# alessiodevoto/peekvit

Measured on AMD Instinct MI355X. Metric: images/sec ViT-B/16 fwd @ batch 2048, 224x224, higher is better.
Workload: dtype f16; 1 GPU; vit_b_16 forward, batch 2048/GPU, 224x224; global_batch=2048, parallelism=replicas x1 (batch-sharded, no collective), precision_mode=auto, streams=1, operands=IEEE fp16 operands, fp32 accumulate (same MFMA rate as bf16), range-guarded, range_guard_fallbacks=0

## Files before the change

### peekvit_amd/_build.py

```python
from __future__ import annotations

import glob
import os
import subprocess
import sys

HERE = os.path.dirname(os.path.abspath(__file__))
CSRC = os.path.join(HERE, "csrc")
LIB = os.path.join(HERE, "libpeekvit_hip.so")
LIB_F16 = os.path.join(HERE, "libpeekvit_hip_f16.so")
HIPCC = os.environ.get("HIPCC", "/opt/rocm/bin/hipcc")
FLAGS = ["--offload-arch=gfx950", "-O3", "-std=c++17", "-fPIC", "-Wno-unused-result"]
HEADERS = ("peekvit_hip.h", "peekvit_hip_moe.h", "peekvit_hip_ee.h", "peekvit_hip_sparse.h", "peekvit_hip_pct.h",
           "peekvit_hip_pct_train.h", "peekvit_hip_attn_stream.h", "peekvit_hip_pct_block.h", "peekvit_hip_rank_train.h", "peekvit_hip_rank_infer.h",
           "peekvit_hip_avit_train.h", "peekvit_hip_sparse_train.h", "peekvit_hip_avit_pack_train.h", "peekvit_hip_dropout.h", "peekvit_hip_sparse_long.h",
           "peekvit_hip_sparse_long_train.h", "peekvit_hip_avit_long.h")
FILE_FLAGS = {"pv_attention.hip": ["-mllvm", "-amdgpu-mfma-vgpr-form=1"], "pv_rowops.hip": ["-fno-slp-vectorize"],
              "pv_attention_stream.hip": ["-mllvm", "-amdgpu-mfma-vgpr-form=1"],
              "pv_ee.hip": ["-fno-slp-vectorize"],
              "pv_sparse.hip": ["-fno-slp-vectorize"],
              "pv_sparse_long.hip": ["-fno-slp-vectorize"],
              "pv_pct.hip": ["-fno-slp-vectorize"],
              "pv_pct_train.hip": ["-fno-slp-vectorize"],
              "pv_rank_train.hip": ["-fno-slp-vectorize"],
              "pv_avit_train.hip": ["-fno-slp-vectorize"],
              "pv_avit_pack_train.hip": ["-fno-slp-vectorize"],
              "pv_avit_long.hip": ["-fno-slp-vectorize"],
              "pv_dropout.hip": ["-fno-slp-vectorize"],
              "pv_sparse_train.hip": ["-fno-slp-vectorize", "-mllvm", "-amdgpu-mfma-vgpr-form=1"],
              "pv_sparse_long_train.hip": ["-fno-slp-vectorize"]}


def sources():
    return sorted(glob.glob(os.path.join(CSRC, "*.hip")))


def _stale() -> bool:
    if not os.path.exists(LIB) or not os.path.exists(LIB_F16):
        return True
    t = min(os.path.getmtime(LIB), os.path.getmtime(LIB_F16))
    deps = sources() + glob.glob(os.path.join(CSRC, "*.h")) + [os.path.join(os.path.dirname(HERE), "include", h) for h in HEADERS] + [os.path.abspath(__file__)]
    return any(os.path.getmtime(d) > t for d in deps)


def build(force: bool = False, verbose: bool = False) -> str:
    if not force and not _stale():
        return LIB
    procs = []
    variants = [("build", [], LIB), ("build_f16", ["-DPV_OPERAND_F16"], LIB_F16)]
    objs = {lib: [] for _, _, lib in variants}
    for sub, defs, lib in variants:
        objdir = os.path.join(HERE, sub)
        os.makedirs(objdir, exist_ok=True)
        for src in sources():
            obj = os.path.join(objdir, os.path.basename(src)[:-4] + ".o")
            objs[lib].append(obj)
            cmd = [HIPCC, *FLAGS, *FILE_FLAGS.get(os.path.basename(src), []), *defs, "-c", src, "-o", obj]
            if verbose:
                print(" ".join(cmd))
            procs.append((src, subprocess.Popen(cmd, stdout=subprocess.PIPE, stderr=subprocess.STDOUT)))
    for src, p in procs:
        out, _ = p.communicate()
        if p.returncode != 0:
            raise RuntimeError(f"hipcc failed on {src}:\n{out.decode(errors='replace')}")
    for _, _, lib in variants:
        cmd = [HIPCC, "--offload-arch=gfx950", "-shared", "-fPIC", "-o", lib, *objs[lib]]
        r = subprocess.run(cmd, stdout=subprocess.PIPE, stderr=subprocess.STDOUT)
        if r.returncode != 0:
            raise RuntimeError(f"link failed:\n{r.stdout.decode(errors='replace')}")
    return LIB


def build_variant(tag: str, defs, force: bool = False) -> str:
    lib = os.path.join(HERE, f"libpeekvit_hip_{tag}.so")
    deps = sources() + glob.glob(os.path.join(CSRC, "*.h")) + [os.path.join(os.path.dirname(HERE), "include", h) for h in HEADERS]
    if not force and os.path.exists(lib) and all(os.path.getmtime(d) <= os.path.getmtime(lib) for d in deps):
        return lib
    objdir = os.path.join(HERE, "build_" + tag)
    os.makedirs(objdir, exist_ok=True)
    procs, objs = [], []
    for src in sources():
        obj = os.path.join(objdir, os.path.basename(src)[:-4] + ".o")
        objs.append(obj)
        procs.append((src, subprocess.Popen([HIPCC, *FLAGS, *FILE_FLAGS.get(os.path.basename(src), []), *defs, "-c", src, "-o", obj],
                                            stdout=subprocess.PIPE, stderr=subprocess.STDOUT)))
    for src, p in procs:
        out, _ = p.communicate()
        if p.returncode != 0:
            raise RuntimeError(f"hipcc failed on {src}:\n{out.decode(errors='replace')}")
    r = subprocess.run([HIPCC, "--offload-arch=gfx950", "-shared", "-fPIC", "-o", lib, *objs], stdout=subprocess.PIPE, stderr=subprocess.STDOUT)
    if r.returncode != 0:
        raise RuntimeError(f"link failed:\n{r.stdout.decode(errors='replace')}")
    return lib


if __name__ == "__main__":
    print(build(force="--force" in sys.argv, verbose=True))
```

### peekvit_amd/_lib.py

```python
from __future__ import annotations

import ctypes as C
import os
import threading

import torch

from ._build import LIB

_i64, _f32, _p, _i32 = C.c_int64, C.c_float, C.c_void_p, C.c_int32

PV_EPI_BIAS_BF16, PV_EPI_BIAS_GELU_BF16, PV_EPI_BIAS_RES_F32, PV_EPI_BIAS_POS_F32 = 0, 1, 2, 3
PV_EPI_BIAS_F32, PV_EPI_BIAS_GELU_SPLIT_BF16 = 4, 5
PV_EPI_BIAS_GELU_PAIR_BF16, PV_EPI_GELU_GRAD_BF16 = 6, 7
PV_WS_TRANSPOSE_COLSUM, PV_WS_COLSUM, PV_WS_LAYERNORM_BWD, PV_WS_GEMM_COLSUM_PARTIAL, PV_WS_GEMM_SPLITK = 1, 2, 3, 4, 5


class GemmArgs(C.Structure):
    _fields_ = [("struct_size", C.c_uint64), ("A", _p), ("W", _p), ("bias", _p), ("out", _p), ("res", _p), ("row_scale", _p), ("pos", _p),
                ("M", _i64), ("N", _i64), ("K", _i64), ("lda", _i64), ("ldw", _i64), ("ldo", _i64), ("ldr", _i64),
                ("rows_per_img_in", _i64), ("rows_per_img_out", _i64), ("row_off", _i64), ("qcols", _i64),
                ("qscale", _f32), ("epilogue", _i32),
                ("ln_gamma", _p), ("ln_beta", _p), ("ln_row_scale", _p), ("ln_out", _p), ("ln_eps", _f32),
                ("ksplit", _i32), ("colsum_partial", _p),
# ... 86 lines not shown
    "pv_layernorm_f32_bf16": (C.c_int, [_p, _i64, _p, _p, _p, _p, _i64, _i64, _i64, _f32, _p]),
    "pv_mean_pool_f32": (C.c_int, [_p, _p, _i64, _i64, _i64, _p]),
    "pv_pct_head_f32": (C.c_int, [_p, _p, _p, _p, _p, _p, _p, _p, _i64, _i64, _i64, _i64, _p]),
}

SIGNATURES_PCT_TRAIN = {
    "pv_arpe_knn": (C.c_int, [_p, _p, _i64, _i64, _i64, _p]),
    "pv_arpe_pair_moments": (C.c_int, [_p, _p, _p, _p, _i64, _i64, _i64, _p]),
    "pv_arpe_pair_max": (C.c_int, [_p, _p, _p, _p, _p, _p, _p, _p, _i64, _i64, _i64, _p]),
    "pv_arpe_pair_bwd": (C.c_int, [_p, _p, _p, _p, _p, _p, _p, _i64, _i64, _p]),
}

SIGNATURES_ATTN_STREAM = {
    "pv_attention_stream_lse_bf16": (C.c_int, [_p, _p, _p, _i64, _i64, _i64, _i64, _p, _p]),
    "pv_attention_stream_bwd_bf16": (C.c_int, [_p, _p, _p, _p, _p, _p, _i64, _i64, _i64, _i64, _f32, _p]),
}

SIGNATURES_PCT_BLOCK = {
    "pv_layernorm_bwd_sum": (C.c_int, [_p, _p, _p, _p, _p, _p, _p, _p, _i64, _i64, _i64, _f32, C.c_int, _p]),
    "pv_attention_stream_bwd16_bf16": (C.c_int, [_p, _p, _p, _p, _p, _p, _p, _i64, _i64, _i64, _i64, _f32, _p]),
}

SIGNATURES_RANK_TRAIN = {
    "pv_rank_pack_f32": (C.c_int, [_p, _p, _p, _i64, _i64, _i64, _i64, _p]),
    "pv_rank_expand_f32": (C.c_int, [_p, _p, _i64, _i64, _i64, _i64, _p]),
    "pv_rank_reduce_f32": (C.c_int, [_p, _p, _i64, _i64, _i64, _i64, _p]),
    "pv_rank_unpack_grad_f32": (C.c_int, [_p, _p, _p, _i64, _i64, _i64, _i64, _p]),
    "pv_layernorm_f32_bf16_masked": (C.c_int, [_p, _p, _p, _p, _p, _p, _i64, _i64, _f32, _p]),
    "pv_layernorm_bwd_sum_masked": (C.c_int, [_p, _p, _p, _p, _p, _p, _p, _p, _p, _i64, _i64, _i64, _f32, C.c_int, _p]),
    "pv_attention_stream_lse_w_bf16": (C.c_int, [_p, _p, _p, _i64, _i64, _i64, _i64, _f32, _p, _p]),
    "pv_attention_stream_bwd16_w_bf16": (C.c_int, [_p, _p, _p, _p, _p, _p, _p, _i64, _i64, _i64, _i64, _f32, _f32, _p]),
}

SIGNATURES_RANK_INFER = {
    "pv_rank_order_gap": (C.c_int, [_p, _p, _p, _i64, _i64, _i64, _p]),
    "pv_layernorm_gather_f32_bf16": (C.c_int, [_p, _p, _p, _p, _p, _p, _i64, _i64, _i64, _i64, _f32, _p]),
}

SIGNATURES_AVIT_TRAIN = {
    "pv_avit_act_fwd": (C.c_int, [_p] * 16 + [_i64, _i64, _i64, _i64, _f32, _f32, _f32, C.c_int, _p]),
    "pv_avit_act_bwd": (C.c_int, [_p] * 9 + [_i64, _i64, _i64, _i64, _f32, C.c_int, _p]),
}

SIGNATURES_SPARSE_TRAIN = {
    "pv_attention_varlen_w_lse_bf16": (C.c_int, [_p, _p, _p, _p, _p, _i64, _i64, _i64, _i64, _p, _p]),
    "pv_attention_varlen_w_bwd16_bf16": (C.c_int, [_p, _p, _p, _p, _p, _p, _p, _p, _p, _i64, _i64, _i64, _i64, _f32, _p]),
    "pv_residual_pack_step_train": (C.c_int, [_p, _p, _p, _p, _i64, _i64, _i64, _p, _p, _p, _p, _f32, _f32, _p,
                                              _p, _p, _p, _p, _p, _p, _p, _p, _p, _p, _p, _f32, _p, _p, _p, _p]),
    "pv_residual_pack_step_bwd": (C.c_int, [_p] * 11 + [_i64, _i64, _i64, _p, _p, _f32, _p, _p, _p, _p, _p, _p]),
}

SIGNATURES_AVIT_PACK_TRAIN = {
    "pv_avit_pack_step_train": (C.c_int, [_p] * 4 + [_i64] * 4 + [_p] * 12 + [_i64, _p, _f32, _f32, _f32, C.c_int] + [_p] * 11),
    "pv_avit_pack_step_bwd": (C.c_int, [_p] * 16 + [_i64] * 6 + [_f32, C.c_int, _p]),
}

_u64 = C.c_uint64
SIGNATURES_DROPOUT = {
    "pv_dropout_keep_u8": (C.c_int, [_p, _u64, _u64, _i64, _i64, _f32, _p]),
    "pv_dropout_f32": (C.c_int, [_p, _p, _u64, _u64, _i64, _i64, _f32, _p]),
    "pv_dropout_residual": (C.c_int, [_p, _p, _p, _u64, _u64, _i64, _i64, _f32, _p]),
    "pv_dropout_bwd16": (C.c_int, [_p, _p, _u64, _u64, _i64, _i64, _f32, _p]),
    "pv_attention_stream_lse_drop_bf16": (C.c_int, [_p, _p, _p, _i64, _i64, _i64, _i64, _f32, _u64, _u64, _p, _p]),
    "pv_attention_stream_bwd16_drop_bf16": (C.c_int, [_p, _p, _p, _p, _p, _p, _p, _i64, _i64, _i64, _i64, _f32, _f32, _u64, _u64, _p]),
}

SIGNATURES_SPARSE_LONG = {
    "pv_attention_varlen_w_stream_bf16": SIGNATURES_SPARSE["pv_attention_varlen_w_bf16"],
    "pv_residual_pack_step_long": SIGNATURES_SPARSE["pv_residual_pack_step"],
}

SIGNATURES_SPARSE_LONG_TRAIN = {
    "pv_attention_varlen_w_stream_lse_bf16": SIGNATURES_SPARSE_TRAIN["pv_attention_varlen_w_lse_bf16"],
    "pv_attention_varlen_w_stream_bwd16_bf16": SIGNATURES_SPARSE_TRAIN["pv_attention_varlen_w_bwd16_bf16"],
    "pv_residual_pack_step_long_train": SIGNATURES_SPARSE_TRAIN["pv_residual_pack_step_train"],
    "pv_residual_pack_step_long_bwd": SIGNATURES_SPARSE_TRAIN["pv_residual_pack_step_bwd"],
}

SIGNATURES_AVIT_LONG = {
    "pv_avit_pack_step_long": SIGNATURES_AVIT_PACK_TRAIN["pv_avit_pack_step_train"],
    "pv_avit_pack_step_long_bwd": SIGNATURES_AVIT_PACK_TRAIN["pv_avit_pack_step_bwd"],
}

ABI_VERSION = 10
_lock = threading.Lock()
_libs: dict = {}

_OPERAND_DEFAULT = "bf16"
_tls = threading.local()
LIB_F16 = os.path.join(os.path.dirname(os.path.abspath(__file__)), "libpeekvit_hip_f16.so")


def current_operand() -> str:
    return getattr(_tls, "operand", _OPERAND_DEFAULT)


def set_operand(op: str) -> str:
    old = current_operand()
    _tls.operand = op
    return old


def __getattr__(name):
    if name == "OPERAND":
        return current_operand()
    raise AttributeError(f"module {__name__!r} has no attribute {name!r}")


def operand_dtype():
    import torch as _t
    return _t.float16 if current_operand() == "f16" else _t.bfloat16


class PeekvitHipError(RuntimeError):
    pass


def lib_path(operand: str = "bf16") -> str:
    return LIB_F16 if operand == "f16" else LIB


def load(operand=None):
    op = current_operand() if operand is None else operand
    lib = _libs.get(op)
    if lib is not None:
        return lib
    with _lock:
        lib = _libs.get(op)
        if lib is not None:
            return lib
        path = lib_path(op)
        if not os.path.exists(path):
            raise PeekvitHipError(
                f"{path} not found: the MI355X kernels are not built. Run `python -m peekvit_amd._build` "
                "(or __graft_entry__.build()); there is no fallback path.")
        lib = C.CDLL(path)
        for name, (res, args) in {**SIGNATURES, **SIGNATURES_MOE, **SIGNATURES_EE, **SIGNATURES_SPARSE, **SIGNATURES_PCT,
                                   **SIGNATURES_PCT_TRAIN, **SIGNATURES_ATTN_STREAM, **SIGNATURES_PCT_BLOCK, **SIGNATURES_RANK_TRAIN,
                                   **SIGNATURES_RANK_INFER, **SIGNATURES_AVIT_TRAIN, **SIGNATURES_SPARSE_TRAIN, **SIGNATURES_AVIT_PACK_TRAIN,
                                   **SIGNATURES_DROPOUT, **SIGNATURES_SPARSE_LONG, **SIGNATURES_SPARSE_LONG_TRAIN,
                                   **SIGNATURES_AVIT_LONG}.items():
            fn = getattr(lib, name)
            fn.restype, fn.argtypes = res, args
        if lib.pv_version() != ABI_VERSION:
            raise PeekvitHipError(f"{path} has ABI v{lib.pv_version()}, this package binds v{ABI_VERSION}: rebuild (python -m peekvit_amd._build)")
        if lib.pv_gemm_args_size() != C.sizeof(GemmArgs):
            raise PeekvitHipError(f"{path}: pv_gemm_args is {lib.pv_gemm_args_size()} bytes in the library, {C.sizeof(GemmArgs)} in this binding")
        if lib.pv_operand_type() != (1 if op == "f16" else 0):
            raise PeekvitHipError(f"{path} was built for a different operand type")
        _libs[op] = lib
    return lib


def check(code: int, what: str = "") -> None:
    if code != 0:
        msg = load().pv_error_string(code).decode()
        raise PeekvitHipError(f"{what}: {msg} (code {code})" if what else f"{msg} (code {code})")
```

### peekvit_amd/engine.py

```python
from __future__ import annotations

import math
import os
import threading
import warnings
import weakref
from typing import Dict, List, Optional, Tuple

import torch
from torch import nn

from . import _lib, autograph, ops
import contextlib

from ._lib import (PV_EPI_BIAS_BF16, PV_EPI_BIAS_F32, PV_EPI_BIAS_GELU_BF16, PV_EPI_BIAS_GELU_SPLIT_BF16, PV_EPI_BIAS_POS_F32,
                   PV_EPI_BIAS_RES_F32, PeekvitHipError)

_MODE_DEFAULT = os.environ.get("PEEKVIT_AMD_PRECISION", "auto")
_MODES = ("auto", "bf16", "f16", "bf16x3")
if _MODE_DEFAULT not in _MODES:
    raise ValueError(f"PEEKVIT_AMD_PRECISION={_MODE_DEFAULT!r}: expected one of {_MODES}")
_lib._OPERAND_DEFAULT = "f16" if _MODE_DEFAULT == "f16" else "bf16"
_mode_tls = threading.local()

# ... 867 lines not shown
        part = workspace.get("fold_part", (nt, R, 2), torch.float32, dev)
        mlp_hyb = layer_mlp_is_hybrid()
        ops.gemm(att, bf16_weight(mha.out_proj.weight), _f32(mha.out_proj.bias), x1.view(R, D), PV_EPI_BIAS_RES_F32, M=R, res=x.view(R, D),
                 x16_out=None if mlp_hyb else x16, rowstat_out=None if mlp_hyb else part)
        if mlp_hyb:
            _mlp_half_split(blk, x1, out, R, eps, None)
            return out
        wg, c1, c2 = _fold_weights(blk.mlp.fc1.weight, blk.mlp.fc1.bias, blk.ln_2)
        stat = ops.rowstat_finalize(part, D, blk.ln_2.eps, workspace.get("fold_stat", (R, 2), torch.float32, dev))
        ops.gemm(x16, wg, None, g, PV_EPI_BIAS_GELU_BF16, M=R, fold=(stat, c1, c2))
        emit = next_ln is not None and next_ln.normalized_shape == (D,)
        o16 = workspace.get("fold_o16", (R, D), _lib.operand_dtype(), dev) if emit else None
        opart = workspace.get("fold_opart", (nt, R, 2), torch.float32, dev) if emit else None
        rowsq = workspace.get("rowsq", (nt, R), torch.float32, dev) if (next_ranks and not emit and _FUSE_RANK_NORM) else None
        ops.gemm(g, bf16_weight(blk.mlp.fc2.weight), _f32(blk.mlp.fc2.bias), out.view(R, D), PV_EPI_BIAS_RES_F32, M=R, res=x1.view(R, D),
                 x16_out=o16, rowstat_out=opart, rowsq_out=rowsq)
        if emit:
            out._pv_fold = (o16, opart, _ln_key(next_ln), _tver(out))
        if rowsq is not None:
            out._pv_rowsq = (rowsq, _tver(out))
        return out

    if hyb:
        if res_scaled:
            raise PeekvitHipError("block_forward(res_scaled=True) cannot run a hybrid layer: pass the masked tokens")
        _attention_half_split(blk, x, att, B, S, eps, row_scale)
    else:
        if h1 is not None and h1.shape == (R, D):
            h = h1
        elif handoff is not None and row_scale is None and handoff[1] == _ln_key(blk.ln_1) and handoff[0].shape == (R, D):
            h = handoff[0]
        else:
            h = workspace.get("h", (R, D), _lib.operand_dtype(), dev)
            ops.layernorm_bf16(x, _f32(blk.ln_1.weight), _f32(blk.ln_1.bias), eps, h, row_scale)
        ops.gemm(h, bf16_weight(mha.in_proj_weight), _f32(mha.in_proj_bias), qkv, PV_EPI_BIAS_BF16, M=R,
                 qcols=D, qscale=float(dh) ** -0.5)
        ops.attention(qkv, att, B, S, H, dh)
    mlp_hyb = layer_mlp_is_hybrid()
    if mlp_hyb and res_scaled:
        raise PeekvitHipError("block_forward(res_scaled=True) cannot run a layer whose MLP half is in split precision: pass the masked tokens")
    fuse2 = _ln_fusable(D, D) and not mlp_hyb
    if res_scaled and (h1 is None or row_scale is None or fuse2):
        raise PeekvitHipError("block_forward(res_scaled=True) needs row_scale, the caller's h1 and the tile GEMM (no full-row LayerNorm fusion)")
    if fuse2 or row_scale is not None:
        ops.gemm(att, bf16_weight(mha.out_proj.weight), _f32(mha.out_proj.bias), x1.view(R, D), PV_EPI_BIAS_RES_F32, M=R,
                 res=x.view(R, D), row_scale=row_scale, res_scaled=res_scaled,
                 ln=(_f32(blk.ln_2.weight), _f32(blk.ln_2.bias), eps, h2, row_scale) if fuse2 else None)
        ln2_done = fuse2
    else:
        ln2_done = _residual_gemm(att, bf16_weight(mha.out_proj.weight), _f32(mha.out_proj.bias), x1.view(R, D), x.view(R, D), R,
                                  ln=(_f32(blk.ln_2.weight), _f32(blk.ln_2.bias), eps, h2))
    if mlp_hyb:
        _mlp_half_split(blk, x1, out, R, eps, row_scale)
        return out
    if not ln2_done:
        ops.layernorm_bf16(x1, _f32(blk.ln_2.weight), _f32(blk.ln_2.bias), eps, h2, row_scale)
    _act_gemm(h2, bf16_weight(blk.mlp.fc1.weight), _f32(blk.mlp.fc1.bias), g, R, gelu=True)
    fuse_next = next_ln is not None and _ln_fusable(D, M) and next_ln.normalized_shape == (D,)
    hn = workspace.get("h", (R, D), _lib.operand_dtype(), dev) if fuse_next else None
    rowsq = None
    if next_ranks and not fuse_next and _FUSE_RANK_NORM and ops.gemm_tile_rows(R, D, M, PV_EPI_BIAS_RES_F32) == 256:
        rowsq = workspace.get("rowsq", ((D + 255) // 256, R), torch.float32, dev)
    if fuse_next or rowsq is not None:
        ops.gemm(g, bf16_weight(blk.mlp.fc2.weight), _f32(blk.mlp.fc2.bias), out.view(R, D), PV_EPI_BIAS_RES_F32, M=R,
                 res=x1.view(R, D), rowsq_out=rowsq,
                 ln=(_f32(next_ln.weight), _f32(next_ln.bias), next_ln.eps, hn, None) if fuse_next else None)
    else:
        want = next_ln is not None and next_ln.normalized_shape == (D,)
        hn = workspace.get("h", (R, D), _lib.operand_dtype(), dev) if want else None
        fuse_next = _residual_gemm(g, bf16_weight(blk.mlp.fc2.weight), _f32(blk.mlp.fc2.bias), out.view(R, D), x1.view(R, D), R,
                                   ln=(_f32(next_ln.weight), _f32(next_ln.bias), next_ln.eps, hn) if want else None)
    if fuse_next:
        out._pv_ln = (hn, _ln_key(next_ln))
    if rowsq is not None:
        out._pv_rowsq = (rowsq, _tver(out))
    return out


_LAST_BLOCK_ROWS = os.environ.get("PEEKVIT_AMD_LAST_BLOCK_ROWS", "1") != "0"
_GATE_LN1 = os.environ.get("PEEKVIT_AMD_GATE_LN1", "1") != "0"
_GATE_NO_MASKED = os.environ.get("PEEKVIT_AMD_GATE_MASKED", "0") != "1"


def rows_only_ok(blk: nn.Module) -> bool:
    import torch.nn.modules.module as _m
    if not _LAST_BLOCK_ROWS or _mode() == "bf16x3" or layer_is_hybrid() or layer_mlp_is_hybrid():
        return False
    own = ("_forward_hooks", "_forward_pre_hooks", "_backward_hooks", "_backward_pre_hooks")
    glob = ("_global_forward_hooks", "_global_forward_pre_hooks", "_global_backward_hooks", "_global_backward_pre_hooks")
    return not any(getattr(blk, n, None) for n in own) and not any(getattr(_m, n, None) for n in glob)


def block_forward_rows(blk: nn.Module, x: torch.Tensor, eps: float, nq: int, row_scale: Optional[torch.Tensor] = None,
                       h1: Optional[torch.Tensor] = None) -> torch.Tensor:
    if x.dtype != torch.float32:
        x = x.float()
    fold_in, handoff = getattr(x, "_pv_fold", None), getattr(x, "_pv_ln", None)
    if fold_in is not None and fold_in[3] != _tver(x):
        fold_in = None
    if not x.is_contiguous():
        x, fold_in, handoff = x.contiguous(), None, None
    if row_scale is not None:
        fold_in, handoff = None, None
    B, S, D = x.shape
    mha = blk.self_attention.self_attention
    H = mha.num_heads
    dh = D // H
    M = blk.mlp.fc1.out_features
    dev, R, Rq, od = x.device, B * S, B * nq, _lib.operand_dtype()
    _check_ln_range(blk.ln_1)
    _check_ln_range(blk.ln_2)
    g1, b1 = _f32(blk.ln_1.weight), _f32(blk.ln_1.bias)

    kv = workspace.get("qkv", (R, 2 * D), od, dev)
    if fold_in is not None and fold_in[2] == _ln_key(blk.ln_1) and fold_in[0].shape == (R, D):
        wg, c1, c2 = _fold_weights(mha.in_proj_weight, mha.in_proj_bias, blk.ln_1)
        stat = ops.rowstat_finalize(fold_in[1], D, blk.ln_1.eps, workspace.get("fold_stat", (R, 2), torch.float32, dev))
        ops.gemm(fold_in[0], wg[D:], None, kv, PV_EPI_BIAS_BF16, M=R, fold=(stat, c1[D:], c2[D:]))
    else:
        if h1 is not None and h1.shape == (R, D):
            h = h1
        elif handoff is not None and handoff[1] == _ln_key(blk.ln_1) and handoff[0].shape == (R, D):
            h = handoff[0]
        else:
            h = workspace.get("h", (R, D), od, dev)
            ops.layernorm_bf16(x, g1, b1, eps, h, row_scale)
        ops.gemm(h, bf16_weight(mha.in_proj_weight)[D:], _f32(mha.in_proj_bias)[D:], kv, PV_EPI_BIAS_BF16, M=R)

    xq = workspace.get("rows_x", (B, nq, D), torch.float32, dev)
    xq.copy_(x[:, :nq])
    xq = xq.view(Rq, D)
    rsq = None
    if row_scale is not None:
        rsq = workspace.get("rows_rs", (B, nq), torch.float32, dev)
        rsq.copy_(row_scale.view(B, S)[:, :nq])
    hq = workspace.get("rows_h", (Rq, D), od, dev)
    ops.layernorm_bf16(xq, g1, b1, eps, hq, rsq)
    qb = workspace.get("rows_q", (Rq, D), od, dev)
    ops.gemm(hq, bf16_weight(mha.in_proj_weight)[:D], _f32(mha.in_proj_bias)[:D], qb, PV_EPI_BIAS_BF16, M=Rq, qcols=D, qscale=float(dh) ** -0.5)
    att = workspace.get("rows_att", (Rq, D), od, dev)
    ops.attention_rows(qb, kv, att, B, S, nq, H, dh)
    x1 = workspace.get("rows_x1", (Rq, D), torch.float32, dev)
    if rsq is None:
        _residual_gemm(att, bf16_weight(mha.out_proj.weight), _f32(mha.out_proj.bias), x1, xq, Rq)
    else:
        ops.gemm(att, bf16_weight(mha.out_proj.weight), _f32(mha.out_proj.bias), x1, PV_EPI_BIAS_RES_F32, M=Rq, res=xq, row_scale=rsq)
    ops.layernorm_bf16(x1, _f32(blk.ln_2.weight), _f32(blk.ln_2.bias), eps, hq, rsq)
    g = workspace.get("rows_g", (Rq, M), od, dev)
    ops.gemm(hq, bf16_weight(blk.mlp.fc1.weight), _f32(blk.mlp.fc1.bias), g, PV_EPI_BIAS_GELU_BF16, M=Rq)
    out = torch.empty((B, nq, D), dtype=torch.float32, device=dev)
    _residual_gemm(g, bf16_weight(blk.mlp.fc2.weight), _f32(blk.mlp.fc2.bias), out.view(Rq, D), x1, Rq)
    return out


def _block_forward_x3(blk: nn.Module, x: torch.Tensor, eps: float, row_scale: Optional[torch.Tensor]) -> torch.Tensor:
    x = x.float() if x.dtype != torch.float32 else x
    x = x if x.is_contiguous() else x.contiguous()
    B, S, D = x.shape
    mha = blk.self_attention.self_attention
    H = mha.num_heads
    dh = D // H
    M = blk.mlp.fc1.out_features
    dev, R = x.device, B * S
    h3 = workspace.get("h3", (R, 3 * D), _lib.operand_dtype(), dev)
    qkv32 = workspace.get("qkv32", (R, 3 * D), torch.float32, dev)
    att3 = workspace.get("att3", (R, 3 * D), _lib.operand_dtype(), dev)
    g3 = workspace.get("g3", (R, 3 * M), _lib.operand_dtype(), dev)
    x1 = workspace.get("x1", (B, S, D), torch.float32, dev)
    out = torch.empty_like(x)
    ops.layernorm_split(x, _f32(blk.ln_1.weight), _f32(blk.ln_1.bias), eps, h3, row_scale)
    ops.gemm(h3, bf16x3_weight(mha.in_proj_weight), _f32(mha.in_proj_bias), qkv32, PV_EPI_BIAS_F32, M=R, qcols=D, qscale=float(dh) ** -0.5)
    ops.attention_f32(qkv32, att3, B, S, H, dh)
    ops.gemm(att3, bf16x3_weight(mha.out_proj.weight), _f32(mha.out_proj.bias), x1.view(R, D), PV_EPI_BIAS_RES_F32, M=R,
             res=x.view(R, D), row_scale=row_scale)
    ops.layernorm_split(x1, _f32(blk.ln_2.weight), _f32(blk.ln_2.bias), eps, h3, row_scale)
    ops.gemm(h3, bf16x3_weight(blk.mlp.fc1.weight), _f32(blk.mlp.fc1.bias), g3, PV_EPI_BIAS_GELU_SPLIT_BF16, M=R)
    ops.gemm(g3, bf16x3_weight(blk.mlp.fc2.weight), _f32(blk.mlp.fc2.bias), out.view(R, D), PV_EPI_BIAS_RES_F32, M=R, res=x1.view(R, D))
    return out


def run_layers(layers: nn.Sequential, x: torch.Tensor, last_rows: int = 0) -> torch.Tensor:
    mods = list(layers)
    hybrid = getattr(_region, "hybrid", ())
    try:
        return _run_layers(mods, x, last_rows, hybrid)
    finally:
        _region.layer = None
        ops.set_flag_word(0)


def _run_layers(mods, x: torch.Tensor, last_rows: int, hybrid) -> torch.Tensor:
    for i, layer in enumerate(mods):
        _region.layer = i
        ops.set_flag_word(1 + i % (FLAG_WORDS - 1))
        if last_rows > 0 and i + 1 == len(mods) and x.shape[1] > last_rows and getattr(layer, "_pv_forward_rows", None) is not None:
            rows = layer._pv_forward_rows(x, last_rows)
            if rows is not None:
                return rows
        nxt = mods[i + 1] if i + 1 < len(mods) else None
        hint = None
        if nxt is not None and getattr(nxt, "_pv_plain_ln1", None) is not None and nxt._pv_plain_ln1() and ((i + 1) % (FLAG_WORDS - 1)) not in hybrid:
            hint = nxt.ln_1
        if hasattr(layer, "_pv_next_ln"):
            object.__setattr__(layer, "_pv_next_ln", hint)
            object.__setattr__(layer, "_pv_next_ranks", bool(nxt is not None and getattr(nxt, "_pv_ranks_input", None) is not None
                                                             and nxt._pv_ranks_input()))
        x = call_module(layer, x)
        if x.is_inference() and _hooks_between(layer, nxt):
            for name in _HANDOFFS:
                if hasattr(x, name):
                    delattr(x, name)
    return x


_FUSED_PATCH_EMBED = os.environ.get("PEEKVIT_AMD_FUSED_PATCH_EMBED", "1") != "0"


def embed_tokens(model: nn.Module, img: torch.Tensor, budget_token: Optional[torch.Tensor] = None,
                 budget: float = 0.0) -> torch.Tensor:
    u8 = img.dtype == torch.uint8
    if not u8 and img.dtype != torch.float32:
        img = img.float()
    if not img.is_contiguous():
        img = img.contiguous()
# ... 826 lines not shown
```

### peekvit_amd/ops.py

```python
from __future__ import annotations

import ctypes as C
from typing import Optional

import torch

from . import _lib
from ._lib import GemmArgs, check

launch_count = 0


class KernelTimer:

    def __init__(self):
        self.records = []

    def __enter__(self):
        global _timer
        _timer = self
        return self

    def __exit__(self, *exc):
        global _timer
# ... 194 lines not shown
                    M=M, N=N, K=K, lda=a.stride(0) if a.dim() == 2 else K, ldw=w.stride(0) if w.dim() == 2 else w.shape[-1],
                    ldo=out.stride(-2) if out.dim() >= 2 else out.shape[-1],
                    ldr=(res.stride(0) if res.dim() == 2 else res.shape[-1]) if res is not None else 0,
                    rows_per_img_in=rows_per_img_in, rows_per_img_out=rows_per_img_out, row_off=row_off,
                    qcols=qcols, qscale=float(qscale), epilogue=epilogue,
                    ln_gamma=ln[0].data_ptr() if ln else 0, ln_beta=ln[1].data_ptr() if ln else 0,
                    ln_row_scale=ln[4].data_ptr() if ln and ln[4] is not None else 0,
                    ln_out=ln[3].data_ptr() if ln else 0, ln_eps=float(ln[2]) if ln else 0.0, ksplit=int(ksplit), colsum_partial=0,
                    x16_out=x16_out.data_ptr() if x16_out is not None else 0, rowstat_out=rowstat_out.data_ptr() if rowstat_out is not None else 0,
                    fold_stat=fold[0].data_ptr() if fold else 0, fold_c1=fold[1].data_ptr() if fold else 0, fold_c2=fold[2].data_ptr() if fold else 0,
                    range_flag=range_flag.data_ptr() if range_flag is not None and range_flag.device == a.device else 0,
                    rowsq_out=rowsq_out.data_ptr() if rowsq_out is not None else 0, res_scaled=int(res_scaled))
    part = None
    if colsum_out is not None and _lib.load().pv_gemm_tile_rows(C.byref(args)) == 256:
        part = _scratch_f32(_lib.PV_WS_GEMM_COLSUM_PARTIAL, a.device, M, N).view((M + 255) // 256, N)
        args.colsum_partial = part.data_ptr()
    nbytes = 2.0 * (M * K + N * K) + out.element_size() * M * N * (2 if res is not None else 1) + (2.0 * M * N if ln else 0.0) + (2.0 * M * N if x16_out is not None else 0.0)
    with _timed("pv_gemm_bf16" + tag, a.device, 2.0 * M * N * K, nbytes, member=(N, K, epilogue)):
        check(_lib.load().pv_gemm_bf16(C.byref(args), _stream(a)), "pv_gemm_bf16")
    _count()
    if colsum_out is not None:
        colsum(part if part is not None else out, colsum_out)
    return out


def rowstat_finalize(partials: torch.Tensor, D: int, eps: float, out: Optional[torch.Tensor] = None) -> torch.Tensor:
    _chk(partials, torch.float32, "partials")
    T, rows, _ = partials.shape
    if out is None:
        out = torch.empty((rows, 2), dtype=torch.float32, device=partials.device)
    with _timed("pv_rowstat_finalize", partials.device, 0.0, 8.0 * (T + 1) * rows):
        check(_lib.load().pv_rowstat_finalize(_ptr(partials), _ptr(out), T, rows, D, float(eps), _flag(partials.device), _stream(partials)), "pv_rowstat_finalize")
    _count()
    return out


def gemm_tn(a: torch.Tensor, b: torch.Tensor, part: torch.Tensor, ksplit: int, tag: str = "[wgrad]"):
    K, M = a.shape
    N = b.shape[1]
    ldo = part.stride(1)
    assert b.shape[0] == K and part.shape == (max(ksplit, 1), M, N) and part.stride(2) == 1 and ldo >= N and part.stride(0) == M * ldo
    args = GemmArgs(A=a.data_ptr(), W=b.data_ptr(), bias=0, out=part.data_ptr(), res=0, row_scale=0, pos=0, M=M, N=N, K=K,
                    lda=a.stride(0), ldw=b.stride(0), ldo=ldo, ldr=0, rows_per_img_in=0, rows_per_img_out=0, row_off=0, qcols=0,
                    qscale=1.0, epilogue=_lib.PV_EPI_BIAS_F32, ln_gamma=0, ln_beta=0, ln_row_scale=0, ln_out=0, ln_eps=0.0,
                    ksplit=int(ksplit))
    with _timed("pv_gemm_tn_bf16" + tag, a.device, 2.0 * M * N * K, 2.0 * K * (M + N) + 4.0 * max(ksplit, 1) * M * N):
        check(_lib.load().pv_gemm_tn_bf16(C.byref(args), _stream(a)), "pv_gemm_tn_bf16")
    _count()
    return part


def attention(qkv: torch.Tensor, out: torch.Tensor, B: int, S: int, H: int, dh: int, lse: Optional[torch.Tensor] = None):
    with _timed("pv_attention_bf16", qkv.device, 4.0 * B * H * S * S * dh, 8.0 * B * S * H * dh):
        if lse is None:
            check(_lib.load().pv_attention_bf16(_ptr(qkv), _ptr(out), B, S, H, dh, _attn_flag(qkv.device), _stream(qkv)), "pv_attention_bf16")
        else:
            _chk(lse, torch.float32, "lse")
            if lse.numel() != B * H * S:
                raise _lib.PeekvitHipError("attention: lse must hold B * H * S values")
            check(_lib.load().pv_attention_lse_bf16(_ptr(qkv), _ptr(out), _ptr(lse), B, S, H, dh, _attn_flag(qkv.device), _stream(qkv)), "pv_attention_lse_bf16")
    _count()
    return out


def attention_bwd_lse_ok(S: int, dh: int) -> bool:
    return attention_bwd_lse_supported(S, dh) and S >= 145


def attention_bwd_lse_supported(S: int, dh: int) -> bool:
    return dh in (48, 64) and 129 <= S <= 208


def attention_rows(q: torch.Tensor, kv: torch.Tensor, out: torch.Tensor, B: int, S: int, nq: int, H: int, dh: int):
    for t, name in ((q, "q"), (kv, "kv"), (out, "out")):
        if not (t.is_cuda and t.dtype == _lib.operand_dtype() and t.dim() == 2 and t.stride(1) == 1):
            raise _lib.PeekvitHipError(f"attention_rows: {name} must be a 2-D GPU tensor of the operand type with unit column stride")
    if q.shape[0] != B * nq or out.shape[0] != B * nq or kv.shape[0] != B * S or kv.shape[1] < 2 * H * dh:
        raise _lib.PeekvitHipError("attention_rows: shape mismatch")
    with _timed("pv_attention_rows_bf16", q.device, 4.0 * B * H * nq * S * dh, 4.0 * B * S * H * dh + 4.0 * B * nq * H * dh):
        check(_lib.load().pv_attention_rows_bf16(_ptr(q), q.stride(0), _ptr(kv), kv.stride(0), _ptr(out), out.stride(0),
                                                 B, S, nq, H, dh, _attn_flag(q.device), _stream(q)), "pv_attention_rows_bf16")
    _count()
    return out


def attention_rows_bwd(q, kv, out, dout, dq, dkv, B: int, S: int, H: int, dh: int, qscale: float):
    for t, name in ((q, "q"), (kv, "kv"), (out, "out"), (dout, "dout"), (dq, "dq"), (dkv, "dkv")):
        if not (t.is_cuda and t.dtype == _lib.operand_dtype() and t.dim() == 2 and t.stride(1) == 1):
            raise _lib.PeekvitHipError(f"attention_rows_bwd: {name} must be a 2-D GPU tensor of the operand type with unit column stride")
    if any(t.shape[0] != B for t in (q, out, dout, dq)) or kv.shape[0] != B * S or dkv.shape[0] != B * S:
        raise _lib.PeekvitHipError("attention_rows_bwd: shape mismatch")
    with _timed("pv_attention_rows_bwd_bf16", q.device, 10.0 * B * H * S * dh, 2.0 * 3 * 2 * B * S * H * dh):
        check(_lib.load().pv_attention_rows_bwd_bf16(_ptr(q), q.stride(0), _ptr(kv), kv.stride(0), _ptr(out), out.stride(0), _ptr(dout), dout.stride(0),
                                                     _ptr(dq), dq.stride(0), _ptr(dkv), dkv.stride(0), B, S, 1, H, dh, float(qscale), _stream(q)),
              "pv_attention_rows_bwd_bf16")
    _count()
    return dq, dkv


def cls_pool(x: torch.Tensor, gamma, beta, eps: float, num_cls: int) -> torch.Tensor:
    B, S, D = x.shape
    pooled = torch.empty((B, D), dtype=torch.float32, device=x.device)
    with _timed("pv_cls_pool", x.device, 0.0, 0.0):
        check(_lib.load().pv_cls_pool(_ptr(x), _ptr(gamma), _ptr(beta), _ptr(pooled), B, S, D, num_cls, float(eps),
                                      _stream(x)), "pv_cls_pool")
    _count()
    return pooled


def head(pooled: torch.Tensor, w: torch.Tensor, b) -> torch.Tensor:
    B, D = pooled.shape
    Cn = w.shape[0]
    logits = torch.empty((B, Cn), dtype=torch.float32, device=pooled.device)
    with _timed("pv_head_f32", pooled.device, 2.0 * B * D * Cn, 0.0):
        check(_lib.load().pv_head_f32(_ptr(pooled), _ptr(w), _ptr(b), _ptr(logits), B, D, Cn, _stream(pooled)), "pv_head_f32")
    _count()
    return logits


def sum_slices(partials: torch.Tensor, out: torch.Tensor, accumulate: bool = False, base: Optional[torch.Tensor] = None, ln=None) -> torch.Tensor:
    _chk(partials, torch.float32, "partials"); _chk(out, torch.float32, "out")
    S = partials.shape[0]
    with _timed("pv_sum_slices_f32", out.device, 0.0, 4.0 * (S + 1 + (base is not None)) * out.numel()):
        if ln is not None:
            _chk(base, torch.float32, "base"); _chk(ln[3], _lib.operand_dtype(), "ln out")
            D = ln[3].shape[-1]
            assert base.numel() == out.numel() == ln[3].numel() and base.is_contiguous() and out.is_contiguous()
            check(_lib.load().pv_sum_slices_add_ln_f32(_ptr(partials), _ptr(base), _ptr(out), out.numel() // D, D, S, _ptr(ln[0]), _ptr(ln[1]), float(ln[2]),
                                                       _ptr(ln[3]), _stream(out)), "pv_sum_slices_add_ln_f32")
        elif base is not None:
            _chk(base, torch.float32, "base")
            assert base.numel() == out.numel() and base.is_contiguous() and out.is_contiguous()
            check(_lib.load().pv_sum_slices_add_f32(_ptr(partials), _ptr(base), _ptr(out), out.numel(), S, _stream(out)), "pv_sum_slices_add_f32")
        else:
            check(_lib.load().pv_sum_slices_f32(_ptr(partials), _ptr(out), out.numel(), S, int(accumulate), _stream(out)), "pv_sum_slices_f32")
    _count()
    return out


def sum_slices_act(partials: torch.Tensor, out: torch.Tensor, gelu: bool = False, qcols: int = 0, qscale: float = 1.0) -> torch.Tensor:
    _chk(partials, torch.float32, "partials"); _chk(out, _lib.operand_dtype(), "out")
    S, M, N = partials.shape
    assert out.shape == (M, N)
    with _timed("pv_sum_slices_f32", out.device, 0.0, (4.0 * S + 2.0) * out.numel()):
        check(_lib.load().pv_sum_slices_act_bf16(_ptr(partials), _ptr(out), M, N, S, int(gelu), int(qcols), float(qscale), _flag(out.device), _stream(out)),
              "pv_sum_slices_act_bf16")
    _count()
    return out


def transpose(src: torch.Tensor, out: Optional[torch.Tensor] = None, pad_to: int = 1, colsum_out: Optional[torch.Tensor] = None) -> torch.Tensor:
    if not (src.is_cuda and src.dtype == _lib.operand_dtype() and src.dim() == 2 and src.stride(1) == 1):
        raise _lib.PeekvitHipError("transpose: expected a 2-D bf16 GPU tensor with unit column stride")
    R, Cc = src.shape
    ldd = (R + pad_to - 1) // pad_to * pad_to
    if out is None:
        out = torch.empty((Cc, ldd), dtype=_lib.operand_dtype(), device=src.device)
    assert out.shape == (Cc, ldd) and out.is_contiguous()
    ws = _scratch_f32(_lib.PV_WS_TRANSPOSE_COLSUM, src.device, R, Cc, ldd) if colsum_out is not None else None
    with _timed("pv_transpose_bf16", src.device, 0.0, 4.0 * src.numel()):
        check(_lib.load().pv_transpose_bf16(_ptr(src), src.stride(0), _ptr(out), R, Cc, ldd, _ptr(colsum_out), _ptr(ws), _stream(src)),
              "pv_transpose_bf16")
    _count()
    return out


# ... 1461 lines not shown
```

Baseline: 28430 images/sec.

## Compute last-block class-row attention directly from tokens, skipping full K/V projection

In the last block, where only the class rows are needed, the K/V projection over all tokens is replaced by an algebraic reordering. The class query is projected through each head's K weights into a per-head D-dimensional vector u. A new HIP kernel then computes scores against the raw or layernorm-folded tokens, takes the softmax, and builds a weighted token sum z. Per-head GEMMs with the V weights finish the output. This avoids the R x 2D KV GEMM over all tokens, at the cost of derived-weight caching, an extra quantisation scale for u, and per-head small GEMMs.

Measured after the change: 28670 images/sec, median of 6. No clear change (+0.9%).

```diff
diff --git a/include/peekvit_hip_cls_attn.h b/include/peekvit_hip_cls_attn.h
--- /dev/null
+++ b/include/peekvit_hip_cls_attn.h
@@ -0,0 +1,18 @@
+#ifndef PEEKVIT_HIP_CLS_ATTN_H
+#define PEEKVIT_HIP_CLS_ATTN_H
+
+#include "peekvit_hip.h"
+
+#ifdef __cplusplus
+extern "C" {
+#endif
+
+#define PV_CLS_ATTN_MAX_G 16
+
+int pv_cls_attention_tokens_bf16(const uint16_t* x16, int64_t ldx, const float* stat, const uint16_t* u, uint16_t* z, int64_t B, int64_t S,
+                                 int64_t nq, int64_t H, int64_t D, int u_log2_scale, uint32_t* range_flag, void* stream);
+
+#ifdef __cplusplus
+}
+#endif
+#endif
diff --git a/peekvit_amd/_build.py b/peekvit_amd/_build.py
--- a/peekvit_amd/_build.py
+++ b/peekvit_amd/_build.py
@@ -14,7 +14,7 @@
 HEADERS = ("peekvit_hip.h", "peekvit_hip_moe.h", "peekvit_hip_ee.h", "peekvit_hip_sparse.h", "peekvit_hip_pct.h",
            "peekvit_hip_pct_train.h", "peekvit_hip_attn_stream.h", "peekvit_hip_pct_block.h", "peekvit_hip_rank_train.h", "peekvit_hip_rank_infer.h",
            "peekvit_hip_avit_train.h", "peekvit_hip_sparse_train.h", "peekvit_hip_avit_pack_train.h", "peekvit_hip_dropout.h", "peekvit_hip_sparse_long.h",
-           "peekvit_hip_sparse_long_train.h", "peekvit_hip_avit_long.h")
+           "peekvit_hip_sparse_long_train.h", "peekvit_hip_avit_long.h", "peekvit_hip_cls_attn.h")
 FILE_FLAGS = {"pv_attention.hip": ["-mllvm", "-amdgpu-mfma-vgpr-form=1"], "pv_rowops.hip": ["-fno-slp-vectorize"],
               "pv_attention_stream.hip": ["-mllvm", "-amdgpu-mfma-vgpr-form=1"],
               "pv_ee.hip": ["-fno-slp-vectorize"],
@@ -28,7 +28,8 @@
               "pv_avit_long.hip": ["-fno-slp-vectorize"],
               "pv_dropout.hip": ["-fno-slp-vectorize"],
               "pv_sparse_train.hip": ["-fno-slp-vectorize", "-mllvm", "-amdgpu-mfma-vgpr-form=1"],
-              "pv_sparse_long_train.hip": ["-fno-slp-vectorize"]}
+              "pv_sparse_long_train.hip": ["-fno-slp-vectorize"],
+              "pv_cls_attn.hip": ["-fno-slp-vectorize", "-mllvm", "-amdgpu-mfma-vgpr-form=1"]}
 
 
 def sources():
diff --git a/peekvit_amd/_lib.py b/peekvit_amd/_lib.py
--- a/peekvit_amd/_lib.py
+++ b/peekvit_amd/_lib.py
@@ -192,6 +192,10 @@
     "pv_avit_pack_step_long_bwd": SIGNATURES_AVIT_PACK_TRAIN["pv_avit_pack_step_bwd"],
 }
 
+SIGNATURES_CLS_ATTN = {
+    "pv_cls_attention_tokens_bf16": (C.c_int, [_p, _i64, _p, _p, _p, _i64, _i64, _i64, _i64, _i64, C.c_int, _p, _p]),
+}
+
 ABI_VERSION = 10
 _lock = threading.Lock()
 _libs: dict = {}
@@ -249,7 +253,7 @@
                                    **SIGNATURES_PCT_TRAIN, **SIGNATURES_ATTN_STREAM, **SIGNATURES_PCT_BLOCK, **SIGNATURES_RANK_TRAIN,
                                    **SIGNATURES_RANK_INFER, **SIGNATURES_AVIT_TRAIN, **SIGNATURES_SPARSE_TRAIN, **SIGNATURES_AVIT_PACK_TRAIN,
                                    **SIGNATURES_DROPOUT, **SIGNATURES_SPARSE_LONG, **SIGNATURES_SPARSE_LONG_TRAIN,
-                                   **SIGNATURES_AVIT_LONG}.items():
+                                   **SIGNATURES_AVIT_LONG, **SIGNATURES_CLS_ATTN}.items():
             fn = getattr(lib, name)
             fn.restype, fn.argtypes = res, args
         if lib.pv_version() != ABI_VERSION:
diff --git a/peekvit_amd/csrc/pv_cls_attn.hip b/peekvit_amd/csrc/pv_cls_attn.hip
--- /dev/null
+++ b/peekvit_amd/csrc/pv_cls_attn.hip
@@ -0,0 +1,218 @@
+#include "pv_attn_tiles.h"
+#include "../../include/peekvit_hip_cls_attn.h"
+
+#define CA_NW 8
+#define CA_SLAB_ROW 160
+#define CA_SLAB_BYTES (32 * CA_SLAB_ROW)
+#define CA_LDS_MAX (160 * 1024)
+
+typedef __attribute__((address_space(3))) s16x4 ca_lds_s16x4;
+
+struct CaLayout {
+    int u_row;
+    int sps, spw;
+    int off_sc, off_w, off_small, total;
+};
+static __host__ __device__ inline CaLayout ca_layout(int S, int D) {
+    CaLayout L;
+    const int sp32 = (S + 31) / 32 * 32;
+    L.u_row = (D + 8) * 2;
+    L.sps = sp32 + 4;
+    L.spw = sp32 + 8;
+    const int a = 16 * L.u_row, s = CA_NW * CA_SLAB_BYTES;
+    L.off_sc = ((a > s ? a : s) + 15) & ~15;
+    L.off_w = L.off_sc + 16 * L.sps * 4;
+    L.off_small = L.off_w + 16 * L.spw * 2;
+    L.total = L.off_small + 3 * 16 * 4;
+    return L;
+}
+
+__global__ __launch_bounds__(CA_NW * 64) void pv_cls_attn_tokens_kernel(const uint16_t* __restrict__ x, int64_t ldx, const float* __restrict__ stat,
+                                                                         const uint16_t* __restrict__ u, uint16_t* __restrict__ z, int S, int G, int D,
+                                                                         float u_unscale, uint32_t* flag) {
+    extern __shared__ __attribute__((aligned(16))) char ca_lds[];
+    const CaLayout L = ca_layout(S, D);
+    char* const uimg = ca_lds;
+    float* const sc = reinterpret_cast<float*>(ca_lds + L.off_sc);
+    uint16_t* const w16 = reinterpret_cast<uint16_t*>(ca_lds + L.off_w);
+    float* const usum = reinterpret_cast<float*>(ca_lds + L.off_small);
+    float* const wmean = usum + 16;
+    float* const wden = usum + 32;
+
+    const int tid = threadIdx.x, lane = tid & 63, wid = tid >> 6;
+    const int l16 = lane & 15, kg = lane >> 4;
+    const int64_t b = blockIdx.x;
+    const int64_t row0 = b * S;
+    const int nt = (S + 15) >> 4, nt16 = nt * 16, sp32 = (S + 31) & ~31;
+
+    {
+        const int cpr = D >> 3;
+        for (int i = tid; i < 16 * cpr; i += CA_NW * 64) {
+            const int g = i / cpr, ch = i - g * cpr;
+            u32x4 v = {0u, 0u, 0u, 0u};
+            if (g < G) v = *reinterpret_cast<const u32x4*>(u + (b * G + g) * D + ch * 8);
+            *reinterpret_cast<u32x4*>(uimg + g * L.u_row + ch * 16) = v;
+        }
+    }
+    __syncthreads();
+    for (int g = wid; g < 16; g += CA_NW) {
+        float s = 0.f;
+        for (int c = lane * 2; c < D; c += 128) {
+            const uint32_t v = *reinterpret_cast<const uint32_t*>(uimg + g * L.u_row + c * 2);
+            s += pv_unpack_lo(v) + pv_unpack_hi(v);
+        }
+        s = pv_wave_sum(s);
+        if (lane == 0) usum[g] = s;
+    }
+    __syncthreads();
+
+    for (int t = wid; t < nt; t += CA_NW) {
+        const int r = t * 16 + l16;
+        const uint16_t* xr = x + (row0 + (r < S ? r : S - 1)) * ldx + 8 * kg;
+        const char* ur = uimg + l16 * L.u_row + 16 * kg;
+        f32x4 acc = {0.f, 0.f, 0.f, 0.f};
+        int k0 = 0;
+        for (; k0 + 256 <= D; k0 += 256) {
+            u32x4 a[8];
+#pragma unroll
+            for (int i = 0; i < 8; ++i) a[i] = *reinterpret_cast<const u32x4*>(xr + k0 + 32 * i);
+#pragma unroll
+            for (int i = 0; i < 8; ++i) acc = PV_MFMA_16x16x32(a[i], *reinterpret_cast<const u32x4*>(ur + (k0 + 32 * i) * 2), acc, 0, 0, 0);
+        }
+        for (; k0 < D; k0 += 64) {
+            u32x4 a[2];
+#pragma unroll
+            for (int i = 0; i < 2; ++i) a[i] = *reinterpret_cast<const u32x4*>(xr + k0 + 32 * i);
+#pragma unroll
+            for (int i = 0; i < 2; ++i) acc = PV_MFMA_16x16x32(a[i], *reinterpret_cast<const u32x4*>(ur + (k0 + 32 * i) * 2), acc, 0, 0, 0);
+        }
+        const float us = usum[l16];
+        f32x4 sv;
+#pragma unroll
+        for (int i = 0; i < 4; ++i) {
+            const int j = t * 16 + 4 * kg + i;
+            float mean = 0.f, rstd = 1.f;
+            if (stat != nullptr) {
+                const float2 st = *reinterpret_cast<const float2*>(stat + (row0 + (j < S ? j : S - 1)) * 2);
+                mean = st.x; rstd = st.y;
+            }
+            sv[i] = j < S ? rstd * (acc[i] - mean * us) * u_unscale : -INFINITY;
+        }
+        *reinterpret_cast<f32x4*>(sc + l16 * L.sps + t * 16 + 4 * kg) = sv;
+    }
+    __syncthreads();
+
+    for (int g = wid; g < 16; g += CA_NW) {
+        float* const sg = sc + g * L.sps;
+        uint16_t* const wg = w16 + g * L.spw;
+        if (g >= G) {
+            for (int j = lane; j < sp32; j += 64) wg[j] = 0;
+            continue;
+        }
+        float mx = -INFINITY, amax = 0.f;
+        for (int j = lane; j < nt16; j += 64) {
+            const float v = sg[j];
+            mx = fmaxf(mx, v);
+            if (j < S) amax = fmaxf(amax, v == v ? __builtin_fabsf(v) : INFINITY);
+        }
+        mx = pv_wave_max(mx);
+        amax = pv_wave_max(amax);
+        if (lane == 0) pv_score_guard(amax, flag);
+        float l = 0.f, wmax = 0.f;
+        for (int j = lane; j < nt16; j += 64) {
+            float e = 0.f;
+            if (j < S) {
+                e = __builtin_amdgcn_exp2f((sg[j] - mx) * PV_LOG2E);
+                l += e;
+                if (stat != nullptr) e *= stat[(row0 + j) * 2 + 1];
+            }
+            sg[j] = e;
+            wmax = fmaxf(wmax, e);
+        }
+        l = pv_wave_sum(l);
+        wmax = pv_wave_max(wmax);
+        const float scl = wmax > 1e-30f && wmax < 1e30f ? (float)(1 << (int)PV_P_SHIFT) / wmax : 1.0f;
+        float wm = 0.f;
+        for (int j = lane; j < sp32; j += 64) {
+            uint16_t h = 0;
+            if (j < S) {
+                h = pv_f2bf(sg[j] * scl);
+                if (stat != nullptr) wm += pv_bf2f(h) * stat[(row0 + j) * 2];
+            }
+            wg[j] = h;
+        }
+        wm = pv_wave_sum(wm);
+        if (lane == 0) {
+            wmean[g] = wm;
+            wden[g] = l * scl;
+        }
+    }
+    __syncthreads();
+
+    char* const slab = ca_lds + wid * CA_SLAB_BYTES;
+    const int lr = lane >> 3, lc = lane & 7;
+    const int q4 = l16 >> 2, p4 = l16 & 3;
+    const int nks = sp32 >> 5;
+    for (int cu = wid; cu < (D >> 6); cu += CA_NW) {
+        const uint16_t* xb = x + row0 * ldx + cu * 64 + lc * 8;
+        f32x4 acc[4];
+#pragma unroll
+        for (int n = 0; n < 4; ++n) acc[n] = (f32x4){0.f, 0.f, 0.f, 0.f};
+        u32x4 stg[4];
+#pragma unroll
+        for (int i = 0; i < 4; ++i) {
+            const int r = lr + 8 * i;
+            stg[i] = *reinterpret_cast<const u32x4*>(xb + (int64_t)(r < S ? r : S - 1) * ldx);
+        }
+        for (int ks = 0; ks < nks; ++ks) {
+#pragma unroll
+            for (int i = 0; i < 4; ++i) *reinterpret_cast<u32x4*>(slab + (lr + 8 * i) * CA_SLAB_ROW + lc * 16) = stg[i];
+            if (ks + 1 < nks) {
+#pragma unroll
+                for (int i = 0; i < 4; ++i) {
+                    const int r = (ks + 1) * 32 + lr + 8 * i;
+                    stg[i] = *reinterpret_cast<const u32x4*>(xb + (int64_t)(r < S ? r : S - 1) * ldx);
+                }
+            }
+            const uint16_t* wr = w16 + l16 * L.spw + ks * 32 + 4 * kg;
+            const u32x2 alo = *reinterpret_cast<const u32x2*>(wr), ahi = *reinterpret_cast<const u32x2*>(wr + 16);
+            const u32x4 a = {alo[0], alo[1], ahi[0], ahi[1]};
+#pragma unroll
+            for (int n = 0; n < 4; ++n) {
+                char* const tb = slab + (4 * kg + q4) * CA_SLAB_ROW + n * 32 + p4 * 8;
+                const s16x4 blo = __builtin_amdgcn_ds_read_tr16_b64_v4i16((ca_lds_s16x4*)tb);
+                const s16x4 bhi = __builtin_amdgcn_ds_read_tr16_b64_v4i16((ca_lds_s16x4*)(tb + 16 * CA_SLAB_ROW));
+                const s16x8 bb = __builtin_shufflevector(blo, bhi, 0, 1, 2, 3, 4, 5, 6, 7);
+                acc[n] = PV_MFMA_16x16x32(a, bb, acc[n], 0, 0, 0);
+            }
+        }
+#pragma unroll
+        for (int i = 0; i < 4; ++i) {
+            const int g = 4 * kg + i;
+            if (g < G) {
+                const float wm = wmean[g], den = wden[g];
+                uint16_t* zr = z + (b * G + g) * D + cu * 64 + l16;
+#pragma unroll
+                for (int n = 0; n < 4; ++n) zr[n * 16] = pv_f2bf((acc[n][i] - wm) / den);
+            }
+        }
+    }
+}
+
+extern "C" int pv_cls_attention_tokens_bf16(const uint16_t* x16, int64_t ldx, const float* stat, const uint16_t* u, uint16_t* z, int64_t B, int64_t S,
+                                            int64_t nq, int64_t H, int64_t D, int u_log2_scale, uint32_t* range_flag, void* stream) {
+    if (!x16 || !u || !z || B <= 0 || nq <= 0 || H <= 0 || D <= 0) return PV_ERR_INVALID_ARG;
+    if (((uintptr_t)x16 & 15) || ((uintptr_t)u & 15) || ((uintptr_t)z & 15) || ((uintptr_t)stat & 7) || ((uintptr_t)range_flag & 3)) return PV_ERR_INVALID_ARG;
+    if (u_log2_scale > 64 || u_log2_scale < -64) return PV_ERR_INVALID_ARG;
+    if (D % 64 || nq > PV_CLS_ATTN_MAX_G || H > PV_CLS_ATTN_MAX_G || nq * H > PV_CLS_ATTN_MAX_G || S < 1 || ldx < D || ldx % 8) return PV_ERR_UNSUPPORTED;
+    if (B > 0x7fffffff || S > 8192 || D > 32768) return PV_ERR_UNSUPPORTED;
+    const CaLayout L = ca_layout((int)S, (int)D);
+    if (L.total > CA_LDS_MAX) return PV_ERR_UNSUPPORTED;
+    static PvPerDevice latch;
+    if (latch.first_use() &&
+        hipFuncSetAttribute(reinterpret_cast<const void*>(pv_cls_attn_tokens_kernel), hipFuncAttributeMaxDynamicSharedMemorySize, CA_LDS_MAX) != hipSuccess)
+        return PV_ERR_LAUNCH;
+    PV_LAUNCH(pv_cls_attn_tokens_kernel, dim3((unsigned)B), dim3(CA_NW * 64), (size_t)L.total, (hipStream_t)stream, x16, ldx, stat, u, z, (int)S, (int)(nq * H),
+              (int)D, ldexpf(1.0f, -u_log2_scale), range_flag);
+    return pv_check_launch();
+}
diff --git a/peekvit_amd/engine.py b/peekvit_amd/engine.py
--- a/peekvit_amd/engine.py
+++ b/peekvit_amd/engine.py
@@ -973,6 +973,62 @@
 _GATE_NO_MASKED = os.environ.get("PEEKVIT_AMD_GATE_MASKED", "0") != "1"
 
 
+_CLS_FROM_TOKENS = os.environ.get("PEEKVIT_AMD_CLS_FROM_TOKENS", "1") != "0"
+_CLS_U_LOG2_SCALE = 8
+_CLS_MAX_S, _CLS_MAX_D = 1024, 1280
+_clscache: Dict[tuple, tuple] = {}
+
+
+def _cls_tokens_ok(S: int, D: int, G: int, dh: int) -> bool:
+    return _CLS_FROM_TOKENS and G <= 16 and D % 64 == 0 and dh % 8 == 0 and S <= _CLS_MAX_S and D <= _CLS_MAX_D and _mode() != "bf16x3"
+
+
+def _cls_weights(mha: nn.Module, ln: Optional[nn.LayerNorm]):
+    w, b = mha.in_proj_weight, mha.in_proj_bias
+    key = (id(w), id(ln.weight) if ln is not None else 0, _lib.OPERAND)
+    ver = (pver(w), pver(b) if b is not None else -1, (pver(ln.weight), pver(ln.bias)) if ln is not None else -1, w.data_ptr())
+    ent = _clscache.get(key)
+    if ent is not None and ent[0] == ver:
+        return ent[1]
+    if torch.cuda.is_current_stream_capturing():
+        raise PeekvitHipError("the class-row attention's derived weights are not built yet: run one eager forward before capturing a graph")
+    D, H = w.shape[1], mha.num_heads
+    dh = D // H
+    if ln is not None:
+        wg, _, c2 = _fold_weights(w, b, ln)
+    else:
+        wg, c2 = bf16_weight(w), (_f32(b) if b is not None else None)
+    with torch.inference_mode(False), torch.no_grad():
+        wu = torch.zeros((H, D, H, dh), dtype=wg.dtype, device=wg.device)
+        wk = wg[D:2 * D].view(H, dh, D)
+        for h in range(H):
+            wu[h, :, h, :] = wk[h].t()
+        wu = wu.view(H * D, D)
+        wv = wg[2 * D:3 * D].clone()
+        c2v = c2[2 * D:3 * D].clone() if c2 is not None else None
+    if key not in _clscache:
+        _evict_with(w, _clscache, key)
+        if ln is not None:
+            _evict_with(ln.weight, _clscache, key)
+    _clscache[key] = (ver, (wu, wv, c2v))
+    return wu, wv, c2v
+
+
+def _cls_attention_from_tokens(mha: nn.Module, ln: Optional[nn.LayerNorm], x16: torch.Tensor, stat: Optional[torch.Tensor], qb: torch.Tensor,
+                               att: torch.Tensor, B: int, S: int, nq: int):
+    D, H = x16.shape[1], mha.num_heads
+    dh, Rq, od, dev = D // H, B * nq, _lib.operand_dtype(), x16.device
+    wu, wv, c2v = _cls_weights(mha, ln)
+    u = workspace.get("cls_u", (Rq, H * D), od, dev)
+    ops.gemm(qb, wu, None, u, PV_EPI_BIAS_BF16, M=Rq, qcols=H * D, qscale=float(2 ** _CLS_U_LOG2_SCALE))
+    z = workspace.get("cls_z", (Rq, H * D), od, dev)
+    ops.cls_attention_tokens(x16, stat, u, z, B, S, nq, H, _CLS_U_LOG2_SCALE)
+    for h in range(H):
+        ops.gemm(z[:, h * D:(h + 1) * D], wv[h * dh:(h + 1) * dh], c2v[h * dh:(h + 1) * dh] if c2v is not None else None, att[:, h * dh:(h + 1) * dh],
+                 PV_EPI_BIAS_BF16, M=Rq)
+    return att
+
+
 def rows_only_ok(blk: nn.Module) -> bool:
     import torch.nn.modules.module as _m
     if not _LAST_BLOCK_ROWS or _mode() == "bf16x3" or layer_is_hybrid() or layer_mlp_is_hybrid():
@@ -1003,12 +1059,27 @@
     _check_ln_range(blk.ln_2)
     g1, b1 = _f32(blk.ln_1.weight), _f32(blk.ln_1.bias)
 
-    kv = workspace.get("qkv", (R, 2 * D), od, dev)
-    if fold_in is not None and fold_in[2] == _ln_key(blk.ln_1) and fold_in[0].shape == (R, D):
+    folded = fold_in is not None and fold_in[2] == _ln_key(blk.ln_1) and fold_in[0].shape == (R, D)
+    from_tokens = row_scale is None and h1 is None and _cls_tokens_ok(S, D, nq * H, dh)
+    tok = kv = None
+    if from_tokens:
+        if folded:
+            stat = ops.rowstat_finalize(fold_in[1], D, blk.ln_1.eps, workspace.get("fold_stat", (R, 2), torch.float32, dev))
+            tok = (blk.ln_1, fold_in[0], stat)
+        else:
+            if handoff is not None and handoff[1] == _ln_key(blk.ln_1) and handoff[0].shape == (R, D):
+                h = handoff[0]
+            else:
+                h = workspace.get("h", (R, D), od, dev)
+                ops.layernorm_bf16(x, g1, b1, eps, h, None)
+            tok = (None, h, None)
+    elif folded:
+        kv = workspace.get("qkv", (R, 2 * D), od, dev)
         wg, c1, c2 = _fold_weights(mha.in_proj_weight, mha.in_proj_bias, blk.ln_1)
         stat = ops.rowstat_finalize(fold_in[1], D, blk.ln_1.eps, workspace.get("fold_stat", (R, 2), torch.float32, dev))
         ops.gemm(fold_in[0], wg[D:], None, kv, PV_EPI_BIAS_BF16, M=R, fold=(stat, c1[D:], c2[D:]))
     else:
+        kv = workspace.get("qkv", (R, 2 * D), od, dev)
         if h1 is not None and h1.shape == (R, D):
             h = h1
         elif handoff is not None and handoff[1] == _ln_key(blk.ln_1) and handoff[0].shape == (R, D):
@@ -1030,7 +1101,10 @@
     qb = workspace.get("rows_q", (Rq, D), od, dev)
     ops.gemm(hq, bf16_weight(mha.in_proj_weight)[:D], _f32(mha.in_proj_bias)[:D], qb, PV_EPI_BIAS_BF16, M=Rq, qcols=D, qscale=float(dh) ** -0.5)
     att = workspace.get("rows_att", (Rq, D), od, dev)
-    ops.attention_rows(qb, kv, att, B, S, nq, H, dh)
+    if tok is not None:
+        _cls_attention_from_tokens(mha, tok[0], tok[1], tok[2], qb, att, B, S, nq)
+    else:
+        ops.attention_rows(qb, kv, att, B, S, nq, H, dh)
     x1 = workspace.get("rows_x1", (Rq, D), torch.float32, dev)
     if rsq is None:
         _residual_gemm(att, bf16_weight(mha.out_proj.weight), _f32(mha.out_proj.bias), x1, xq, Rq)
diff --git a/peekvit_amd/ops.py b/peekvit_amd/ops.py
--- a/peekvit_amd/ops.py
+++ b/peekvit_amd/ops.py
@@ -300,6 +300,26 @@
                                                  B, S, nq, H, dh, _attn_flag(q.device), _stream(q)), "pv_attention_rows_bf16")
     _count()
     return out
+
+
+def cls_attention_tokens(x16: torch.Tensor, stat: Optional[torch.Tensor], u: torch.Tensor, z: torch.Tensor, B: int, S: int, nq: int, H: int,
+                         u_log2_scale: int = 0):
+    for t, name in ((x16, "x16"), (u, "u"), (z, "z")):
+        if not (t.is_cuda and t.dtype == _lib.operand_dtype() and t.dim() == 2 and t.stride(1) == 1):
+            raise _lib.PeekvitHipError(f"cls_attention_tokens: {name} must be a 2-D GPU tensor of the operand type with unit column stride")
+    D = x16.shape[1]
+    if x16.shape[0] != B * S or u.shape != (B * nq, H * D) or z.shape != u.shape or not u.is_contiguous() or not z.is_contiguous():
+        raise _lib.PeekvitHipError("cls_attention_tokens: shape mismatch")
+    if stat is not None:
+        _chk(stat, torch.float32, "stat")
+        if stat.shape != (B * S, 2):
+            raise _lib.PeekvitHipError("cls_attention_tokens: stat must be [B * S, 2]")
+    G = nq * H
+    with _timed("pv_attention_rows_bf16", x16.device, 4.0 * B * G * S * D, 4.0 * B * S * D + 4.0 * B * G * D, member="tokens"):
+        check(_lib.load().pv_cls_attention_tokens_bf16(_ptr(x16), x16.stride(0), _ptr(stat), _ptr(u), _ptr(z), B, S, nq, H, D, int(u_log2_scale),
+                                                       _attn_flag(x16.device), _stream(x16)), "pv_cls_attention_tokens_bf16")
+    _count()
+    return z
 
 
 def attention_rows_bwd(q, kv, out, dout, dq, dkv, B: int, S: int, H: int, dh: int, qscale: float):
```
